# matheusfalcaopinto/triple-hybrid-rag

Measured on AMD Instinct MI355X. Metric: queries/sec (fused top-10), higher is better.
Workload: dtype f16 MFMA shortlist scan (f32 accumulate) + f64 rescoring of the f32 rows; 1 GPU; 1000000-doc / 768-d dense-only brute-force cosine top-10 (BASELINE.json configs[1]); pipeline=dense, docs=1000000, dim=768, semantic_top_k=100, fused_top_k=10, shortlist=f16, parallelism=single GPU, world_size_seen=1, rescued_queries=0

## Files before the change

### triple-hybrid-rag_amd/csrc/dense_scan_f16q.hpp

```cpp
#pragma once
#include "dense_common.hpp"

namespace thr {

constexpr int Q_RING = 4;
constexpr int Q_NW = 4;

template <int DIM>
struct QScan {
    static constexpr int KS = DIM / 16;
    static constexpr int HS = KS / 2;
    static constexpr int HALF_BYTES = HS * 1024;
    static constexpr int PER_CU = DIM <= 768 ? 2 : 1;
    static constexpr int NB = (160 * 1024 / PER_CU) / HALF_BYTES > 4 ? 4 : (160 * 1024 / PER_CU) / HALF_BYTES;
    static constexpr int PER = HS / Q_NW;
#ifndef THR_Q_RING_1024
#define THR_Q_RING_1024 8
#endif
    static constexpr int RING = PER_CU == 1 ? THR_Q_RING_1024 : Q_RING;
#ifdef Q_PROBE_EXTRA
    static constexpr int VM_PER_PIECE = 2, LDS_BYTES = NB * HALF_BYTES + 32 * 1024;
#else
    static constexpr int VM_PER_PIECE = 1, LDS_BYTES = NB * HALF_BYTES;
#endif
    static_assert(HS % Q_NW == 0 && NB >= 3, "half tile must split evenly over the waves; >= 3 buffers");
};

template <int DIM, int SHAPE>
__global__ __launch_bounds__(256) void pack_queries_f16(const float* __restrict__ queries,
                                                        int n_queries, f32x4* __restrict__ qfrag,
                                                        float* __restrict__ qerr) {
    constexpr int KS = DIM / 16;
    const int lane = threadIdx.x & 63, wave = threadIdx.x >> 6;
    __shared__ double red[4][4][32];
    double e = 0.0, nn = 0.0, e_hi = 0.0, n_hi = 0.0;
#pragma unroll 4
    for (int s = wave; s < KS; s += 4) {
        int q, d0;
        if constexpr (SHAPE == 32) {
            q = blockIdx.x * 32 + (lane & 31);
            d0 = 16 * s + 8 * (lane >> 5);
        } else {
            q = blockIdx.x * 32 + 16 * (s / (KS / 2)) + (lane & 15);
            d0 = 32 * (s % (KS / 2)) + 8 * (lane >> 4);
        }
        f32x4 lo = {0.f, 0.f, 0.f, 0.f}, hi = lo;
        if (q < n_queries) {
            const f32x4* src = reinterpret_cast<const f32x4*>(queries + (int64_t)q * DIM + d0);
            lo = src[0];
            hi = src[1];
        }
        const f32x4 packed = pack_f16x8(lo, hi);
        qfrag[((int64_t)blockIdx.x * KS + s) * 64 + lane] = packed;
        const half8 hv = __builtin_bit_cast(half8, packed);
        double e1 = 0.0, n1 = 0.0;
#pragma unroll
        for (int j = 0; j < 8; ++j) {
            const float v = j < 4 ? lo[j] : hi[j - 4];
            const double d = (double)v - (double)(float)hv[j];
            e1 += d * d;
            n1 += (double)v * (double)v;
        }
        if (SHAPE == 32 || s < KS / 2) {
            e += e1;
            nn += n1;
        } else {
            e_hi += e1;
            n_hi += n1;
        }
    }
    if constexpr (SHAPE == 32) {
        e += __shfl_xor(e, 32, WAVE);
        nn += __shfl_xor(nn, 32, WAVE);
        if (lane < 32) {
            red[wave][0][lane] = e;
            red[wave][1][lane] = nn;
        }
    } else {
#pragma unroll
        for (int m = 16; m <= 32; m <<= 1) {
            e += __shfl_xor(e, m, WAVE);
            nn += __shfl_xor(nn, m, WAVE);
            e_hi += __shfl_xor(e_hi, m, WAVE);
            n_hi += __shfl_xor(n_hi, m, WAVE);
        }
        if (lane < 16) {
            red[wave][0][lane] = e;
            red[wave][1][lane] = nn;
            red[wave][0][16 + lane] = e_hi;
            red[wave][1][16 + lane] = n_hi;
        }
    }
    __syncthreads();
    if (threadIdx.x < 32) {
        double es = 0.0, ns = 0.0;
#pragma unroll
        for (int w = 0; w < 4; ++w) {
            es += red[w][0][threadIdx.x];
            ns += red[w][1][threadIdx.x];
        }
        const float rel = ns > 0.0 ? (float)sqrt(es / ns) : 0.f;
        qerr[blockIdx.x * 32 + threadIdx.x] = __uint_as_float(__float_as_uint(rel) + 1u);
    }
}

#define QS_RD(dst, ks) \
    asm volatile("ds_read_b128 %0, %1 offset:%2" : "=v"(dst) : "v"(abase), "n"((ks) * 1024) : "memory")
template <int S, int HS, int RING>
__device__ __forceinline__ void qs_fill(f32x4 (&a)[RING], uint32_t abase) {
    if constexpr (S < RING && S < HS) {
        QS_RD(a[S], S);
        qs_fill<S + 1, HS>(a, abase);
    }
}
template <int SHAPE>
struct QAcc;
template <>
struct QAcc<32> {
    static constexpr int NQL = 1, SEGS = 2;
    static constexpr int QW = 32, NQB = 2, NREG = 16;
    f32x16 v;
    __device__ __forceinline__ void zero() {
#pragma unroll
        for (int x = 0; x < 16; ++x) v[x] = 0.f;
    }
    template <int X> __device__ __forceinline__ float get() const { return v[X]; }
    template <int X> static __device__ __forceinline__ int row(int lane) { return (X & 3) + 8 * (X >> 2) + 4 * (lane >> 5); }
    template <int X> static constexpr int qsel() { return 0; }
    static __device__ __forceinline__ int query(int lane, int) { return lane & 31; }
    static __device__ __forceinline__ int seg(int lane) { return lane >> 5; }
};
template <>
struct QAcc<48> {
    static constexpr int NQL = 3, SEGS = 4;
    static constexpr int QW = 48, NQB = 3, NREG = 24;
    f32x4 t[6];
    __device__ __forceinline__ void zero() {
#pragma unroll
        for (int x = 0; x < 6; ++x) t[x] = f32x4{0.f, 0.f, 0.f, 0.f};
    }
    template <int X> __device__ __forceinline__ float get() const { return t[X >> 2][X & 3]; }
    template <int X> static __device__ __forceinline__ int row(int lane) { return 16 * ((X >> 2) / 3) + 4 * (lane >> 4) + (X & 3); }
    template <int X> static constexpr int qsel() { return (X >> 2) % 3; }
    static __device__ __forceinline__ int query(int lane, int qb) { return 16 * qb + (lane & 15); }
    static __device__ __forceinline__ int seg(int lane) { return lane >> 4; }
};
template <>
struct QAcc<16> {
    static constexpr int NQL = 2, SEGS = 4;
    static constexpr int QW = 32, NQB = 2, NREG = 16;
    f32x4 t[4];
    __device__ __forceinline__ void zero() {
#pragma unroll
        for (int x = 0; x < 4; ++x) t[x] = f32x4{0.f, 0.f, 0.f, 0.f};
    }
    template <int X> __device__ __forceinline__ float get() const { return t[X >> 2][X & 3]; }
    template <int X> static __device__ __forceinline__ int row(int lane) { return 16 * (X >> 3) + 4 * (lane >> 4) + (X & 3); }
    template <int X> static constexpr int qsel() { return (X >> 2) & 1; }
    static __device__ __forceinline__ int query(int lane, int qb) { return 16 * qb + (lane & 15); }
    static __device__ __forceinline__ int seg(int lane) { return lane >> 4; }
};

template <int S, int K0, int KS, int SHAPE, int NBQ>
__device__ __forceinline__ void qsx_mfma(const f32x4& a, const f32x4 (&bq)[NBQ], QAcc<SHAPE>& acc) {
    if constexpr (SHAPE == 32) {
        acc.v = __builtin_amdgcn_mfma_f32_32x32x16_f16(__builtin_bit_cast(half8, a),
                                                       __builtin_bit_cast(half8, bq[K0 + S]), acc.v, 0, 0, 0);
    } else {
        constexpr int k32 = (K0 + S) / 2, ra = S & 1, NQB = QAcc<SHAPE>::NQB;
        static_assert(NBQ == NQB * KS / 2, "one B fragment per 16-query block and 32-dim step");
        static_for<0, NQB>([&](auto qb) {
            acc.t[NQB * ra + qb] = __builtin_amdgcn_mfma_f32_16x16x32_f16(
                __builtin_bit_cast(half8, a), __builtin_bit_cast(half8, bq[qb * (KS / 2) + k32]),
                acc.t[NQB * ra + qb], 0, 0, 0);
        });
    }
}
template <int S, int HS, int K0, int KS, int PER, int SHAPE, int RING, int NBQ, typename Issue>
__device__ __forceinline__ void qsx_steps(f32x4 (&a)[RING], const f32x4 (&bq)[NBQ], QAcc<SHAPE>& acc,
                                          uint32_t abase, Issue& issue_piece) {
    if constexpr (S < HS) {
        constexpr int left = HS - S - 1 < RING - 1 ? HS - S - 1 : RING - 1;
        asm volatile("s_waitcnt lgkmcnt(%1)" : "+v"(a[S % RING]) : "n"(left) : "memory");
        qsx_mfma<S, K0, KS, SHAPE>(a[S % RING], bq, acc);
        if constexpr (S + RING < HS) QS_RD(a[S % RING], S + RING);
        constexpr int every = HS / PER;
        if constexpr (S % every == 1 && S / every < PER) issue_piece(std::integral_constant<int, S / every>{});
        qsx_steps<S + 1, HS, K0, KS, PER, SHAPE, RING, NBQ>(a, bq, acc, abase, issue_piece);
    }
}

template <int NQL, bool COLL>
struct QColl {
    const int32_t* doc_coll;
    int qc[NQL];
};
template <int NQL>
struct QColl<NQL, false> {};

template <int SHAPE, bool COLL>
struct QEmit : QColl<QAcc<SHAPE>::NQL, COLL> {
    static constexpr int NQL = QAcc<SHAPE>::NQL;
    const Cand* cand;
    float tau[NQL];
    uint32_t slot[NQL], end[NQL];
    template <int X>
    __device__ __forceinline__ void one(const QAcc<SHAPE>& acc, uint32_t row0, int lane) {
        constexpr int qs = QAcc<SHAPE>::template qsel<X>();
        const float v = acc.template get<X>();
        if (v >= tau[qs]) {
            const uint32_t row = row0 + (uint32_t)QAcc<SHAPE>::template row<X>(lane);
            if constexpr (COLL) {
                if (this->qc[qs] != -1 && this->doc_coll[row] != this->qc[qs]) return;
            }
            if (slot[qs] < end[qs]) {
                const uint64_t word = (uint64_t)__float_as_uint(v) | ((uint64_t)row << 32);
                asm volatile("global_store_dwordx2 %0, %1, %2" ::"v"(slot[qs]), "v"(word), "s"(cand) : "memory");
            }
            slot[qs] += 8;
        }
    }
    template <int X>
    __device__ __forceinline__ void all(const QAcc<SHAPE>& acc, uint32_t row0, int lane) {
        if constexpr (X < QAcc<SHAPE>::NREG) {
            one<X>(acc, row0, lane);
            all<X + 1>(acc, row0, lane);
        }
    }
};

template <int SHAPE, bool COLL>
struct QTop : QColl<QAcc<SHAPE>::NQL, COLL> {
    static constexpr int NQL = QAcc<SHAPE>::NQL;
    float t[NQL][SAMPLE_TOP];
    __device__ __forceinline__ void init() {
#pragma unroll
        for (int u = 0; u < NQL; ++u)
#pragma unroll
            for (int j = 0; j < SAMPLE_TOP; ++j) t[u][j] = -INFINITY;
    }
    template <int X>
    __device__ __forceinline__ void one(const QAcc<SHAPE>& acc, uint32_t row0, int lane) {
        constexpr int qs = QAcc<SHAPE>::template qsel<X>();
        float x = acc.template get<X>();
        x = x == x ? x : -INFINITY;
        if constexpr (COLL) {
            if (this->doc_coll && this->qc[qs] != -1 && x > -INFINITY) {
                const uint32_t row = row0 + (uint32_t)QAcc<SHAPE>::template row<X>(lane);
                if (this->doc_coll[row] != this->qc[qs]) x = -INFINITY;
            }
        }
#pragma unroll
        for (int j = 0; j < SAMPLE_TOP; ++j) {
            const float hi = fmaxf(t[qs][j], x);
            x = fminf(t[qs][j], x);
            t[qs][j] = hi;
        }
    }
    template <int X>
    __device__ __forceinline__ void all(const QAcc<SHAPE>& acc, uint32_t row0, int lane) {
        if constexpr (X < QAcc<SHAPE>::NREG) {
            one<X>(acc, row0, lane);
            all<X + 1>(acc, row0, lane);
        }
    }
    __device__ __forceinline__ void store(float* __restrict__ sample, int u, int64_t q, int nseg, int seg) const {
        float* dst = sample + (q * nseg + seg) * SAMPLE_TOP;
#pragma unroll
        for (int j = 0; j < SAMPLE_TOP; ++j) dst[j] = t[u][j];
    }
};

template <int S, int HS, int K0, int KS, int PER, int SHAPE, int HF, int RING, int NBQ, bool COLL, typename Issue>
__device__ __forceinline__ void qsx_steps_pe(f32x4 (&a)[RING], const f32x4 (&bq)[NBQ], QAcc<SHAPE>& acc,
                                             uint32_t abase, Issue& issue_piece, QEmit<SHAPE, COLL>& em,
                                             const QAcc<SHAPE>& prv, uint32_t row_prv, int lane) {
    if constexpr (S < HS) {
        constexpr int left = HS - S - 1 < RING - 1 ? HS - S - 1 : RING - 1;
        asm volatile("s_waitcnt lgkmcnt(%1)" : "+v"(a[S % RING]) : "n"(left) : "memory");
        qsx_mfma<S, K0, KS, SHAPE>(a[S % RING], bq, acc);
        if constexpr (S + RING < HS) QS_RD(a[S % RING], S + RING);
        constexpr int every = HS / PER;
        if constexpr (S % every == 1 && S / every < PER) issue_piece(std::integral_constant<int, S / every>{});
        constexpr int NRH = QAcc<SHAPE>::NREG / 2, j = S * NRH / HS;
        if constexpr ((S + 1) * NRH / HS > j) em.template one<NRH * HF + j>(prv, row_prv, lane);
        qsx_steps_pe<S + 1, HS, K0, KS, PER, SHAPE, HF, RING, NBQ, COLL>(a, bq, acc, abase, issue_piece, em, prv, row_prv, lane);
    }
}
#undef QS_RD

template <int DIM, int MODE, bool PROF = false, int SHAPE = 32, bool COLL = true>
__global__ __launch_bounds__(Q_NW * 64, QScan<DIM>::PER_CU) void dense_scan_f16q(
    const f32x4* __restrict__ packed, const f32x4* __restrict__ qfrag, int n_qtiles,
    int64_t n_tiles, int64_t tile_stride, const float* __restrict__ tau,
    int* __restrict__ seg_cnt, Cand* __restrict__ cand, int seg_cap,
    float* __restrict__ sample,
    const int32_t* __restrict__ doc_coll, const int32_t* __restrict__ query_coll, int n_queries,
    unsigned long long* __restrict__ stamps = nullptr) {
    using C = QScan<DIM>;
    using A = QAcc<SHAPE>;
    constexpr int KS = C::KS, HS = C::HS, NB = C::NB, PER = C::PER, NQL = A::NQL, QW = A::QW;
    constexpr int NBQ = SHAPE == 32 ? KS : A::NQB * KS / 2;
    extern __shared__ f32x4 lds_rows[];

    const ScanSlot slot = scan_slot(n_qtiles);
    const int lane = threadIdx.x & 63;
    const int wave = __builtin_amdgcn_readfirstlane(threadIdx.x >> 6);
    const int q32 = slot.qtile * Q_NW + wave;
    const bool idle = (int64_t)q32 * QW >= n_queries;

    f32x4 bq[NBQ];
    if (!idle)
        static_for<0, NBQ>([&](auto s) {
            bq[s] = qfrag[((int64_t)q32 * NBQ + s) * 64 + lane];
        });
    const int nseg = A::SEGS * slot.nslices;
    const int my_seg = A::SEGS * slot.slice + A::seg(lane);
    QEmit<SHAPE, COLL> em;
    em.cand = cand;
    QTop<SHAPE, COLL> top;
    if constexpr (COLL) em.doc_coll = top.doc_coll = doc_coll;
    top.init();
    uint32_t start[NQL];
#pragma unroll
    for (int u = 0; u < NQL; ++u) {
        const int q = q32 * QW + A::query(lane, u);
        em.tau[u] = MODE == MODE_FILTER ? tau[q] : 0.f;
        if constexpr (COLL) em.qc[u] = top.qc[u] = (query_coll && q < n_queries) ? query_coll[q] : -1;
        start[u] = (uint32_t)(((int64_t)q * CAND_CAP + (int64_t)my_seg * seg_cap) * sizeof(Cand));
        em.slot[u] = start[u];
        em.end[u] = start[u] + (uint32_t)(seg_cap * sizeof(Cand));
    }
    __builtin_amdgcn_s_waitcnt(0x0F70);

    const int64_t first = slot.slice, step = slot.nslices;
    const int64_t n_mine = first < n_tiles ? (n_tiles - first + step - 1) / step : 0;
    const int64_t n_half = 2 * n_mine;
    const uint32_t lds_base = (uint32_t)(size_t)(__attribute__((address_space(3))) void*)lds_rows;
    auto piece_src = [&](int64_t j) -> const f32x4* {
        const int64_t jc = j < n_half ? j : n_half - 1;
        const int64_t t = first + (jc >> 1) * step;
        return packed + ((t * tile_stride * KS + (jc & 1) * HS + wave) * 64 + lane);
    };
#ifdef Q_PROBE_EXTRA
    f32x4 probe_reg = {0.f, 0.f, 0.f, 0.f};
#endif
    auto dma = [&](const f32x4* src, int buf, int p) {
        __builtin_amdgcn_global_load_lds(
            (const __attribute__((address_space(1))) void*)(src + p * Q_NW * 64),
            (__attribute__((address_space(3))) void*)(size_t)(lds_base + buf * C::HALF_BYTES +
                                                              (wave + p * Q_NW) * 1024),
            16, 0, 0);
#ifdef Q_PROBE_EXTRA
        const uint32_t scratch = lds_base + NB * C::HALF_BYTES + (wave + (p & 7) * Q_NW) * 1024;
        if constexpr (Q_PROBE_EXTRA == 1) {
            __builtin_amdgcn_global_load_lds(
                (const __attribute__((address_space(1))) void*)(src + p * Q_NW * 64),
                (__attribute__((address_space(3))) void*)(size_t)scratch, 16, 0, 0);
        } else {
            asm volatile("ds_write_b128 %0, %1" ::"v"(scratch + lane * 16), "v"(probe_reg) : "memory");
            asm volatile("global_load_dwordx4 %0, %1, off" : "=v"(probe_reg) : "v"(src + p * Q_NW * 64) : "memory");
        }
#endif
    };
    if (n_half > 0) {
#pragma unroll
        for (int b = 0; b < NB - 1; ++b) {
            const f32x4* src = piece_src(b);
#pragma unroll
            for (int p = 0; p < PER; ++p) dma(src, b, p);
        }
    }

    unsigned long long ph[5] = {0, 0, 0, 0, 0}, t_loop = 0, t_prev = 0;
    auto stamp = [&](int j) {
        if constexpr (PROF) {
            const unsigned long long t = __builtin_amdgcn_s_memtime();
            if (j >= 0) ph[j] += t - t_prev;
            t_prev = t;
        }
    };
    if constexpr (PROF) t_loop = __builtin_amdgcn_s_memtime();

    A acc;
    int buf = 0;
    if (idle) {
#pragma unroll 1
        for (int64_t j = 0; j < n_half; ++j) {
            asm volatile("s_waitcnt vmcnt(%0)" ::"n"((NB - 2) * PER * C::VM_PER_PIECE) : "memory");
            __builtin_amdgcn_s_barrier();
            const int nbuf = buf == 0 ? NB - 1 : buf - 1;
            const f32x4* src = piece_src(j + NB - 1);
#pragma unroll
            for (int p = 0; p < PER; ++p) dma(src, nbuf, p);
            buf = buf + 1 == NB ? 0 : buf + 1;
        }
    }
#ifdef Q_NO_PIPE_EMIT
    constexpr bool PIPE_EMIT = false;
#else
    constexpr bool PIPE_EMIT = true;
#endif
    if constexpr (PIPE_EMIT && MODE == MODE_FILTER && !PROF && C::PER_CU == 1 && SHAPE != 48) {
        A acc2[2];
#pragma unroll
        for (int x = 0; x < A::NREG; ++x) {
            if constexpr (SHAPE == 32) acc2[1].v[x] = -INFINITY;
            else acc2[1].t[x >> 2][x & 3] = -INFINITY;
        }
        uint32_t row_of[2] = {0u, 0u};
#define QS_HALF_PE(hf, CUR, PRV)                                                                   \
    {                                                                                              \
        asm volatile("s_waitcnt vmcnt(%0)" ::"n"((NB - 2) * PER * C::VM_PER_PIECE) : "memory");                      \
        __builtin_amdgcn_s_barrier();                                                              \
        const int nbuf = buf == 0 ? NB - 1 : buf - 1;                  \
        const f32x4* src = piece_src(2 * i + (hf) + NB - 1);                                       \
        auto issue_piece = [&](auto P) { dma(src, nbuf, decltype(P)::value); };                    \
        const uint32_t abase = lds_base + buf * C::HALF_BYTES + lane * 16;                         \
        f32x4 a[C::RING];                                                                           \
        qs_fill<0, HS>(a, abase);                                                                  \
        qsx_steps_pe<0, HS, (hf) * HS, KS, PER, SHAPE, (hf)>(a, bq, acc2[CUR], abase, issue_piece, \
                                                            em, acc2[PRV], row_of[PRV], lane);     \
        buf = buf + 1 == NB ? 0 : buf + 1;                                                         \
    }
        const int64_t n_it = idle ? 0 : n_mine;
        int64_t i = 0;
#pragma unroll 1
        for (; i + 1 < n_it; i += 2) {
            acc2[0].zero();
            QS_HALF_PE(0, 0, 1)
            QS_HALF_PE(1, 0, 1)
            row_of[0] = (uint32_t)((first + i * step) * tile_stride * 32);
            ++i;
            acc2[1].zero();
            QS_HALF_PE(0, 1, 0)
            QS_HALF_PE(1, 1, 0)
            row_of[1] = (uint32_t)((first + i * step) * tile_stride * 32);
            --i;
        }
        if (i < n_it) {
            acc2[0].zero();
            QS_HALF_PE(0, 0, 1)
            QS_HALF_PE(1, 0, 1)
            em.template all<0>(acc2[0], (uint32_t)((first + i * step) * tile_stride * 32), lane);
        } else if (n_it > 0) {
            em.template all<0>(acc2[1], row_of[1], lane);
        }
#undef QS_HALF_PE
    } else {
#pragma unroll 1
    for (int64_t i = 0; i < (idle ? 0 : n_mine); ++i) {
#define QS_HALF(hf)                                                                                \
    {                                                                                              \
        stamp(-1);                                                                                 \
               \
        asm volatile("s_waitcnt vmcnt(%0)" ::"n"((NB - 2) * PER * C::VM_PER_PIECE) : "memory");                      \
        stamp(0);                                                                                  \
        __builtin_amdgcn_s_barrier();                                                              \
        stamp(1);                                                                                  \
        const int nbuf = buf == 0 ? NB - 1 : buf - 1;                  \
        const f32x4* src = piece_src(2 * i + (hf) + NB - 1);                                       \
        auto issue_piece = [&](auto P) { dma(src, nbuf, decltype(P)::value); };                    \
        const uint32_t abase = lds_base + buf * C::HALF_BYTES + lane * 16;                         \
        f32x4 a[C::RING];                                                                           \
        qs_fill<0, HS>(a, abase);                                                                  \
        stamp(2);                                                                                  \
        qsx_steps<0, HS, (hf) * HS, KS, PER, SHAPE>(a, bq, acc, abase, issue_piece);                \
        if constexpr (PROF) {                                                                      \
            if constexpr (SHAPE == 32) asm volatile("" : "+v"(acc.v));                               \
            else {                                                                                 \
                asm volatile("" : "+v"(acc.t[0]), "+v"(acc.t[1]), "+v"(acc.t[2]), "+v"(acc.t[3]));   \
                if constexpr (A::NQB == 3) asm volatile("" : "+v"(acc.t[4]), "+v"(acc.t[5]));       \
            }                                                                                      \
        }                                                                                          \
        stamp(3);                                                                                  \
        buf = buf + 1 == NB ? 0 : buf + 1;                                                         \
    }
        acc.zero();
        QS_HALF(0)
        QS_HALF(1)
#undef QS_HALF

        const int64_t t = first + i * step;
        if constexpr (MODE == MODE_ALL) {
            top.template all<0>(acc, (uint32_t)(t * tile_stride * 32), lane);
        } else {
            em.template all<0>(acc, (uint32_t)(t * tile_stride * 32), lane);
        }
        stamp(4);
    }
    }
    asm volatile("s_waitcnt vmcnt(0)" ::: "memory");
    if constexpr (MODE == MODE_FILTER) {
#pragma unroll
        for (int u = 0; u < NQL; ++u)
            seg_cnt[(int64_t)(q32 * QW + A::query(lane, u)) * nseg + my_seg] = (int)((em.slot[u] - start[u]) / sizeof(Cand));
    } else {
#pragma unroll
        for (int u = 0; u < NQL; ++u) top.store(sample, u, (int64_t)q32 * QW + A::query(lane, u), nseg, my_seg);
    }
    if constexpr (PROF) {
        if (lane == 0) {
            unsigned long long* o = stamps + ((int64_t)blockIdx.x * Q_NW + wave) * 8;
            for (int j = 0; j < 5; ++j) o[j] = ph[j];
            o[5] = (unsigned long long)n_half;
            o[6] = __builtin_amdgcn_s_memtime() - t_loop;
            o[7] = (unsigned long long)__builtin_amdgcn_s_getreg((4 << 0) | (0 << 6) | (31 << 11));
        }
    }
}

constexpr int QS_NW = 8;
constexpr int QS_NBUF = 6;

template <int DIM>
struct QStag {
    static constexpr int KS = DIM / 16, HS = KS / 2, HALF_BYTES = HS * 1024;
    static constexpr int PER = HS / QS_NW;
    static constexpr int LDS_BYTES = QS_NBUF * HALF_BYTES;
    static_assert(HS % QS_NW == 0 && LDS_BYTES <= 160 * 1024, "dim 512 / 768 only");
};

template <int DIM, int MODE, int SHAPE = 32, bool COLL = true>
__global__ __launch_bounds__(QS_NW * 64) void dense_scan_f16qs(
    const f32x4* __restrict__ packed, const f32x4* __restrict__ qfrag, int n_qtiles,
    int64_t n_tiles, int64_t tile_stride, const float* __restrict__ tau,
    int* __restrict__ seg_cnt, Cand* __restrict__ cand, int seg_cap,
    float* __restrict__ sample,
    const int32_t* __restrict__ doc_coll, const int32_t* __restrict__ query_coll, int n_queries) {
    using C = QStag<DIM>;
    using A = QAcc<SHAPE>;
    constexpr int KS = C::KS, HS = C::HS, PER = C::PER, NBUF = QS_NBUF, NQL = A::NQL;
    extern __shared__ f32x4 lds_rows[];

    const ScanSlot slot = scan_slot(n_qtiles);
    const int lane = threadIdx.x & 63;
    const int wave = __builtin_amdgcn_readfirstlane(threadIdx.x >> 6);
    const int q32 = slot.qtile * QS_NW + wave;

    f32x4 bq[KS];
    if ((int64_t)q32 * 32 < n_queries)
        static_for<0, KS>([&](auto s) {
            bq[s] = qfrag[((int64_t)q32 * KS + s) * 64 + lane];
        });
    const int nseg = A::SEGS * slot.nslices;
    const int my_seg = A::SEGS * slot.slice + A::seg(lane);
    QEmit<SHAPE, COLL> em;
    em.cand = cand;
    QTop<SHAPE, COLL> top;
    if constexpr (COLL) em.doc_coll = top.doc_coll = doc_coll;
    top.init();
    uint32_t start[NQL];
#pragma unroll
    for (int u = 0; u < NQL; ++u) {
        const int q = q32 * 32 + A::query(lane, u);
        em.tau[u] = MODE == MODE_FILTER ? tau[q] : 0.f;
        if constexpr (COLL) em.qc[u] = top.qc[u] = (query_coll && q < n_queries) ? query_coll[q] : -1;
        start[u] = (uint32_t)(((int64_t)q * CAND_CAP + (int64_t)my_seg * seg_cap) * sizeof(Cand));
        em.slot[u] = start[u];
        em.end[u] = start[u] + (uint32_t)(seg_cap * sizeof(Cand));
    }
    __builtin_amdgcn_s_waitcnt(0x0F70);

    const int64_t first = slot.slice, step = slot.nslices;
    const int64_t n_mine = first < n_tiles ? (n_tiles - first + step - 1) / step : 0;
    const int64_t n_half = 2 * n_mine;
    const uint32_t lds_base = (uint32_t)(size_t)(__attribute__((address_space(3))) void*)lds_rows;
    auto piece_src = [&](int64_t j) -> const f32x4* {
        const int64_t jc = j < n_half ? j : n_half - 1;
        const int64_t t = first + (jc >> 1) * step;
        return packed + ((t * tile_stride * KS + (jc & 1) * HS + wave) * 64 + lane);
    };
    auto dma = [&](const f32x4* src, int buf, int p) {
        __builtin_amdgcn_global_load_lds(
            (const __attribute__((address_space(1))) void*)(src + p * QS_NW * 64),
            (__attribute__((address_space(3))) void*)(size_t)(lds_base + buf * C::HALF_BYTES +
                                                              (wave + p * QS_NW) * 1024),
            16, 0, 0);
    };
#define QS_EMIT(i_)                                                                                \
    if constexpr (MODE == MODE_ALL) {                                                              \
        top.template all<0>(acc, (uint32_t)((first + (i_) * step) * tile_stride * 32), lane);      \
    } else {                                                                                       \
        em.template all<0>(acc, (uint32_t)((first + (i_) * step) * tile_stride * 32), lane);       \
    }
#define QS_SYNC()                                                      \
    asm volatile("s_waitcnt vmcnt(%0)" ::"n"(3 * PER) : "memory");     \
    __builtin_amdgcn_s_barrier();

    if (n_half > 0) {
#pragma unroll
        for (int b = 0; b < 4; ++b) {
            const f32x4* src = piece_src(b);
#pragma unroll
            for (int p = 0; p < PER; ++p) dma(src, b, p);
        }
    }
    A acc;
    f32x4 a[Q_RING];
    if ((int64_t)q32 * 32 >= n_queries) {
        int buf = wave < 4 ? 4 : 5;
        int64_t j = wave < 4 ? 4 : 5;
        if (wave >= 4) {
            QS_SYNC()
            if (n_half > 0) {
                const f32x4* src = piece_src(4);
#pragma unroll
                for (int p = 0; p < PER; ++p) dma(src, 4, p);
            }
        }
#pragma unroll 1
        for (int64_t k = 0; k < n_half; ++k, ++j) {
            QS_SYNC()
            const f32x4* src = piece_src(j);
#pragma unroll
            for (int p = 0; p < PER; ++p) dma(src, buf, p);
            buf = buf + 1 == NBUF ? 0 : buf + 1;
        }
        if (wave < 4) {
            QS_SYNC()
        }
    } else if (wave < 4) {
        int buf = 0;
#pragma unroll 1
        for (int64_t i = 0; i < n_mine; ++i) {
            {
                QS_SYNC()
                const int nbuf = buf + 4 >= NBUF ? buf + 4 - NBUF : buf + 4;
                const f32x4* src = piece_src(2 * i + 4);
                auto issue_piece = [&](auto P) { dma(src, nbuf, decltype(P)::value); };
                const uint32_t abase = lds_base + buf * C::HALF_BYTES + lane * 16;
                qs_fill<0, HS>(a, abase);
                acc.zero();
                qsx_steps<0, HS, 0, KS, PER, SHAPE>(a, bq, acc, abase, issue_piece);
                buf = buf + 1 == NBUF ? 0 : buf + 1;
            }
            {
                QS_SYNC()
                const int nbuf = buf + 4 >= NBUF ? buf + 4 - NBUF : buf + 4;
                const f32x4* src = piece_src(2 * i + 5);
                auto issue_piece = [&](auto P) { dma(src, nbuf, decltype(P)::value); };
                const uint32_t abase = lds_base + buf * C::HALF_BYTES + lane * 16;
                qs_fill<0, HS>(a, abase);
                qsx_steps<0, HS, HS, KS, PER, SHAPE>(a, bq, acc, abase, issue_piece);
                buf = buf + 1 == NBUF ? 0 : buf + 1;
            }
            QS_EMIT(i)
        }
        QS_SYNC()
    } else {
        QS_SYNC()
        if (n_half > 0) {
            const f32x4* src = piece_src(4);
#pragma unroll
            for (int p = 0; p < PER; ++p) dma(src, 4, p);
        }
        int buf = 0;
#pragma unroll 1
        for (int64_t i = 0; i < n_mine; ++i) {
            const int buf1 = buf + 1 == NBUF ? 0 : buf + 1;
            const int buf2 = buf1 + 1 == NBUF ? 0 : buf1 + 1;
            {
                QS_SYNC()
                if (i > 0) {
                    QS_EMIT(i - 1)
                }
                const int nbuf = buf + 5 >= NBUF ? buf + 5 - NBUF : buf + 5;
                const f32x4* src = piece_src(2 * i + 5);
                auto issue_piece = [&](auto P) { dma(src, nbuf, decltype(P)::value); };
                const uint32_t abase = lds_base + buf * C::HALF_BYTES + lane * 16;
                if (i == 0) qs_fill<0, HS>(a, abase);
                acc.zero();
                qsx_steps<0, HS, 0, KS, PER, SHAPE>(a, bq, acc, abase, issue_piece);
                qs_fill<0, HS>(a, lds_base + buf1 * C::HALF_BYTES + lane * 16);
            }
            {
                QS_SYNC()
                const f32x4* src = piece_src(2 * i + 6);
                auto issue_piece = [&](auto P) { dma(src, buf, decltype(P)::value); };
                const uint32_t abase = lds_base + buf1 * C::HALF_BYTES + lane * 16;
                qsx_steps<0, HS, HS, KS, PER, SHAPE>(a, bq, acc, abase, issue_piece);
                if (i + 1 < n_mine)
                    qs_fill<0, HS>(a, lds_base + buf2 * C::HALF_BYTES + lane * 16);
            }
            buf = buf2;
        }
        if (n_mine > 0) {
            QS_EMIT(n_mine - 1)
        }
    }
#undef QS_SYNC
#undef QS_EMIT
    asm volatile("s_waitcnt vmcnt(0)" ::: "memory");
    if constexpr (MODE == MODE_FILTER) {
#pragma unroll
        for (int u = 0; u < NQL; ++u)
            seg_cnt[(int64_t)(q32 * 32 + A::query(lane, u)) * nseg + my_seg] = (int)((em.slot[u] - start[u]) / sizeof(Cand));
    } else {
#pragma unroll
        for (int u = 0; u < NQL; ++u) top.store(sample, u, (int64_t)q32 * 32 + A::query(lane, u), nseg, my_seg);
    }
}

__global__ __launch_bounds__(256) void quantize_f16_norm(const float* __restrict__ docs,
                                                         int64_t n_docs, int dim, int shape,
                                                         _Float16* __restrict__ packed,
                                                         unsigned int* __restrict__ max_err_bits) {
    const int lane = threadIdx.x & 63;
    const int64_t row = (int64_t)blockIdx.x * (blockDim.x / WAVE) + (threadIdx.x >> 6);
    const int64_t n_pad = (n_docs + 31) / 32 * 32;
    if (row >= n_pad) return;
    const int64_t tile = row >> 5;
    const int r = (int)(row & 31), ks = dim / 16;
    const float* x = docs + row * dim;
    double nn = 0.0;
    if (row < n_docs)
        for (int i = lane; i < dim; i += WAVE) nn += (double)x[i] * (double)x[i];
    for (int m = 32; m >= 1; m >>= 1) nn += __shfl_xor(nn, m, WAVE);
    const double dn = sqrt(nn);
    const bool live = dn > 0.0;
    double err = 0.0;
    for (int i = lane; i < dim; i += WAVE) {
        const float v = live ? x[i] : 0.f;
        const _Float16 hv = live ? (_Float16)(float)((double)v / dn) : (_Float16)__builtin_nanf("");
        if (packed) {
            if (shape == 32) {
                const int s = i >> 4, hh = (i >> 3) & 1, e = i & 7;
                packed[(((tile * ks + s) * 64) + r + 32 * hh) * 8 + e] = hv;
            } else {
                const int k32 = i >> 5, g = (i >> 3) & 3, e = i & 7, ra = r >> 4;
                packed[(((tile * ks + 2 * k32 + ra) * 64) + (r & 15) + 16 * g) * 8 + e] = hv;
            }
        }
        if (live) {
            const double d = (double)v / dn - (double)(float)hv;
            err += d * d;
        }
    }
    for (int m = 32; m >= 1; m >>= 1) err += __shfl_xor(err, m, WAVE);
    if (lane == 0 && live) {
        float rel = (float)sqrt(err);
        rel = __uint_as_float(__float_as_uint(rel) + 1u);
        atomicMax(max_err_bits, __float_as_uint(rel));
    }
}

__global__ __launch_bounds__(256) void measure_f16_error(const float* __restrict__ docs, int64_t n_docs,
                                                         int dim, unsigned int* __restrict__ max_rel_bits) {
    const int lane = threadIdx.x & 63;
    const int64_t row = (int64_t)blockIdx.x * (blockDim.x / WAVE) + (threadIdx.x >> 6);
    if (row >= n_docs) return;
    const float* x = docs + row * dim;
    double err = 0.0, nrm = 0.0;
    for (int i = lane; i < dim; i += WAVE) {
        const float v = x[i];
        const double d = (double)v - (double)(float)(_Float16)v;
        err += d * d;
        nrm += (double)v * (double)v;
    }
    for (int m = 32; m >= 1; m >>= 1) {
        err += __shfl_xor(err, m, WAVE);
        nrm += __shfl_xor(nrm, m, WAVE);
    }
    if (lane == 0 && nrm > 0.0) {
        float rel = (float)sqrt(err / nrm);
        rel = __uint_as_float(__float_as_uint(rel) + 1u);
        atomicMax(max_rel_bits, __float_as_uint(rel));
    }
}

}
```

Before: 790,900 queries/s.

## Restructure staggered f16 scan around whole-tile buffers with dedicated issuer waves

Reworks the 8-wave staggered scan kernel so each LDS buffer holds a whole tile instead of a half, with one barrier per tile instead of two. Only waves 4-7 issue global-to-LDS DMA, spreading the pieces across their MFMA steps, while waves 0-3 only multiply. The schedule (buffer count, prologue depth, vmcnt wait depth) moves into a new constexpr helper header. This halves barrier count and simplifies buffer rotation, at the cost of fewer LDS buffers (4 full tiles vs 6 halves) and an uneven DMA load between wave groups.

```diff
diff --git a/triple-hybrid-rag_amd/csrc/dense_scan_f16q.hpp b/triple-hybrid-rag_amd/csrc/dense_scan_f16q.hpp
--- a/triple-hybrid-rag_amd/csrc/dense_scan_f16q.hpp
+++ b/triple-hybrid-rag_amd/csrc/dense_scan_f16q.hpp
@@ -1,5 +1,6 @@
 #pragma once
 #include "dense_common.hpp"
+#include "dense_tile_schedule.hpp"
 
 namespace thr {
 
@@ -285,6 +286,19 @@
         constexpr int NRH = QAcc<SHAPE>::NREG / 2, j = S * NRH / HS;
         if constexpr ((S + 1) * NRH / HS > j) em.template one<NRH * HF + j>(prv, row_prv, lane);
         qsx_steps_pe<S + 1, HS, K0, KS, PER, SHAPE, HF, RING, NBQ, COLL>(a, bq, acc, abase, issue_piece, em, prv, row_prv, lane);
+    }
+}
+template <int S, int KS, int PB, int SHAPE, int RING, int NBQ, typename Issue>
+__device__ __forceinline__ void qst_steps(f32x4 (&a)[RING], const f32x4 (&bq)[NBQ], QAcc<SHAPE>& acc,
+                                          uint32_t abase, Issue& issue_piece) {
+    if constexpr (S < KS) {
+        constexpr int left = KS - S - 1 < RING - 1 ? KS - S - 1 : RING - 1;
+        asm volatile("s_waitcnt lgkmcnt(%1)" : "+v"(a[S % RING]) : "n"(left) : "memory");
+        qsx_mfma<S, 0, KS, SHAPE>(a[S % RING], bq, acc);
+        if constexpr (S + RING < KS) QS_RD(a[S % RING], S + RING);
+        constexpr int p = (S - 1) / 2;
+        if constexpr (S >= 1 && p < PB && tsched::issue_step(p) == S) issue_piece(std::integral_constant<int, p>{});
+        qst_steps<S + 1, KS, PB, SHAPE, RING, NBQ>(a, bq, acc, abase, issue_piece);
     }
 }
 #undef QS_RD
@@ -510,15 +524,16 @@
     }
 }
 
-constexpr int QS_NW = 8;
-constexpr int QS_NBUF = 6;
+constexpr int QS_NW = tsched::N_WAVES;
 
 template <int DIM>
 struct QStag {
-    static constexpr int KS = DIM / 16, HS = KS / 2, HALF_BYTES = HS * 1024;
-    static constexpr int PER = HS / QS_NW;
-    static constexpr int LDS_BYTES = QS_NBUF * HALF_BYTES;
-    static_assert(HS % QS_NW == 0 && LDS_BYTES <= 160 * 1024, "dim 512 / 768 only");
+    static constexpr int KS = tsched::pieces_per_tile(DIM), TILE_BYTES = tsched::tile_bytes(DIM);
+    static constexpr int NBUF = tsched::nbuf(DIM);
+    static constexpr int PB = tsched::pieces_issued(tsched::ROLE_B, DIM);
+    static constexpr int LDS_BYTES = NBUF * TILE_BYTES;
+    static_assert(KS % tsched::N_ISSUERS == 0 && NBUF >= 3 && LDS_BYTES <= tsched::LDS_BUDGET, "dim 512 / 768 only");
+    static_assert(tsched::wait_leaves(tsched::ROLE_B, DIM) < 64 && tsched::issue_step(PB - 1) < KS, "vmcnt is 6 bits");
 };
 
 template <int DIM, int MODE, int SHAPE = 32, bool COLL = true>
@@ -530,7 +545,7 @@
     const int32_t* __restrict__ doc_coll, const int32_t* __restrict__ query_coll, int n_queries) {
     using C = QStag<DIM>;
     using A = QAcc<SHAPE>;
-    constexpr int KS = C::KS, HS = C::HS, PER = C::PER, NBUF = QS_NBUF, NQL = A::NQL;
+    constexpr int KS = C::KS, PB = C::PB, NQL = A::NQL;
     extern __shared__ f32x4 lds_rows[];
 
     const ScanSlot slot = scan_slot(n_qtiles);
@@ -562,20 +577,21 @@
     }
     __builtin_amdgcn_s_waitcnt(0x0F70);
 
+    namespace ts = tsched;
     const int64_t first = slot.slice, step = slot.nslices;
     const int64_t n_mine = first < n_tiles ? (n_tiles - first + step - 1) / step : 0;
-    const int64_t n_half = 2 * n_mine;
     const uint32_t lds_base = (uint32_t)(size_t)(__attribute__((address_space(3))) void*)lds_rows;
+    const ts::Role role = ts::role_of(wave, (int64_t)q32 * 32 >= n_queries);
+    const int iw = wave & (ts::N_ISSUERS - 1);
     auto piece_src = [&](int64_t j) -> const f32x4* {
-        const int64_t jc = j < n_half ? j : n_half - 1;
-        const int64_t t = first + (jc >> 1) * step;
-        return packed + ((t * tile_stride * KS + (jc & 1) * HS + wave) * 64 + lane);
+        const int64_t t = first + ts::source_tile(j, n_mine) * step;
+        return packed + ((t * tile_stride * KS + iw) * 64 + lane);
     };
     auto dma = [&](const f32x4* src, int buf, int p) {
         __builtin_amdgcn_global_load_lds(
-            (const __attribute__((address_space(1))) void*)(src + p * QS_NW * 64),
-            (__attribute__((address_space(3))) void*)(size_t)(lds_base + buf * C::HALF_BYTES +
-                                                              (wave + p * QS_NW) * 1024),
+            (const __attribute__((address_space(1))) void*)(src + (ts::piece_index(iw, p) - iw) * 64),
+            (__attribute__((address_space(3))) void*)(size_t)(lds_base + buf * C::TILE_BYTES +
+                                                              ts::piece_index(iw, p) * 1024),
             16, 0, 0);
     };
 #define QS_EMIT(i_)                                                                                \
@@ -584,112 +600,74 @@
     } else {                                                                                       \
         em.template all<0>(acc, (uint32_t)((first + (i_) * step) * tile_stride * 32), lane);       \
     }
-#define QS_SYNC()                                                      \
-    asm volatile("s_waitcnt vmcnt(%0)" ::"n"(3 * PER) : "memory");     \
+    constexpr int WAIT_B = ts::wait_leaves(ts::ROLE_B, DIM);
+    static_assert(WAIT_B == ts::wait_leaves(ts::ROLE_PAD_B, DIM) && ts::pieces_issued(ts::ROLE_PAD_B, DIM) == PB &&
+                  ts::pieces_issued(ts::ROLE_A, DIM) == 0 && ts::pieces_issued(ts::ROLE_PAD_A, DIM) == 0,
+                  "a padding wave moves what a working wave of its group moves");
+#define QS_SYNC_B()                                                    \
+    asm volatile("s_waitcnt vmcnt(%0)" ::"n"(WAIT_B) : "memory");      \
     __builtin_amdgcn_s_barrier();
 
-    if (n_half > 0) {
-#pragma unroll
-        for (int b = 0; b < 4; ++b) {
+    if (ts::issues(role) && n_mine > 0) {
+#pragma unroll
+        for (int b = 0; b < ts::prologue_tiles(DIM); ++b) {
             const f32x4* src = piece_src(b);
 #pragma unroll
-            for (int p = 0; p < PER; ++p) dma(src, b, p);
+            for (int p = 0; p < PB; ++p) dma(src, ts::buffer_of(b, DIM), p);
         }
     }
     A acc;
     f32x4 a[Q_RING];
-    if ((int64_t)q32 * 32 >= n_queries) {
-        int buf = wave < 4 ? 4 : 5;
-        int64_t j = wave < 4 ? 4 : 5;
-        if (wave >= 4) {
-            QS_SYNC()
-            if (n_half > 0) {
-                const f32x4* src = piece_src(4);
-#pragma unroll
-                for (int p = 0; p < PER; ++p) dma(src, 4, p);
+    auto no_piece = [](auto) {};
+    if (!ts::multiplies(role)) {
+        if (ts::issues(role)) {
+            int ibuf = ts::buffer_of(ts::issue_tile(0, DIM), DIM);
+#pragma unroll 1
+            for (int64_t t = 0; t < ts::barriers(ts::ROLE_PAD_B, n_mine); ++t) {
+                QS_SYNC_B()
+                const f32x4* src = piece_src(ts::issue_tile(t, DIM));
+#pragma unroll
+                for (int p = 0; p < PB; ++p) dma(src, ibuf, p);
+                ibuf = ts::next_buffer(ibuf, DIM);
             }
-        }
+        } else {
 #pragma unroll 1
-        for (int64_t k = 0; k < n_half; ++k, ++j) {
-            QS_SYNC()
-            const f32x4* src = piece_src(j);
-#pragma unroll
-            for (int p = 0; p < PER; ++p) dma(src, buf, p);
-            buf = buf + 1 == NBUF ? 0 : buf + 1;
-        }
-        if (wave < 4) {
-            QS_SYNC()
-        }
-    } else if (wave < 4) {
+            for (int64_t t = 0; t < ts::barriers(ts::ROLE_PAD_A, n_mine); ++t) __builtin_amdgcn_s_barrier();
+        }
+    } else if (role == ts::ROLE_A) {
         int buf = 0;
 #pragma unroll 1
-        for (int64_t i = 0; i < n_mine; ++i) {
-            {
-                QS_SYNC()
-                const int nbuf = buf + 4 >= NBUF ? buf + 4 - NBUF : buf + 4;
-                const f32x4* src = piece_src(2 * i + 4);
-                auto issue_piece = [&](auto P) { dma(src, nbuf, decltype(P)::value); };
-                const uint32_t abase = lds_base + buf * C::HALF_BYTES + lane * 16;
-                qs_fill<0, HS>(a, abase);
-                acc.zero();
-                qsx_steps<0, HS, 0, KS, PER, SHAPE>(a, bq, acc, abase, issue_piece);
-                buf = buf + 1 == NBUF ? 0 : buf + 1;
-            }
-            {
-                QS_SYNC()
-                const int nbuf = buf + 4 >= NBUF ? buf + 4 - NBUF : buf + 4;
-                const f32x4* src = piece_src(2 * i + 5);
-                auto issue_piece = [&](auto P) { dma(src, nbuf, decltype(P)::value); };
-                const uint32_t abase = lds_base + buf * C::HALF_BYTES + lane * 16;
-                qs_fill<0, HS>(a, abase);
-                qsx_steps<0, HS, HS, KS, PER, SHAPE>(a, bq, acc, abase, issue_piece);
-                buf = buf + 1 == NBUF ? 0 : buf + 1;
-            }
+        for (int64_t i = 0; i < ts::barriers(ts::ROLE_A, n_mine); ++i) {
+            __builtin_amdgcn_s_barrier();
+            const uint32_t abase = lds_base + buf * C::TILE_BYTES + lane * 16;
+            qs_fill<0, KS>(a, abase);
+            acc.zero();
+            qst_steps<0, KS, 0, SHAPE>(a, bq, acc, abase, no_piece);
+            buf = ts::next_buffer(buf, DIM);
             QS_EMIT(i)
         }
-        QS_SYNC()
     } else {
-        QS_SYNC()
-        if (n_half > 0) {
-            const f32x4* src = piece_src(4);
-#pragma unroll
-            for (int p = 0; p < PER; ++p) dma(src, 4, p);
-        }
         int buf = 0;
 #pragma unroll 1
-        for (int64_t i = 0; i < n_mine; ++i) {
-            const int buf1 = buf + 1 == NBUF ? 0 : buf + 1;
-            const int buf2 = buf1 + 1 == NBUF ? 0 : buf1 + 1;
-            {
-                QS_SYNC()
-                if (i > 0) {
-                    QS_EMIT(i - 1)
-                }
-                const int nbuf = buf + 5 >= NBUF ? buf + 5 - NBUF : buf + 5;
-                const f32x4* src = piece_src(2 * i + 5);
-                auto issue_piece = [&](auto P) { dma(src, nbuf, decltype(P)::value); };
-                const uint32_t abase = lds_base + buf * C::HALF_BYTES + lane * 16;
-                if (i == 0) qs_fill<0, HS>(a, abase);
-                acc.zero();
-                qsx_steps<0, HS, 0, KS, PER, SHAPE>(a, bq, acc, abase, issue_piece);
-                qs_fill<0, HS>(a, lds_base + buf1 * C::HALF_BYTES + lane * 16);
+        for (int64_t i = 0; i < ts::barriers(ts::ROLE_B, n_mine); ++i) {
+            QS_SYNC_B()
+            if (i > 0) {
+                QS_EMIT(i - 1)
             }
-            {
-                QS_SYNC()
-                const f32x4* src = piece_src(2 * i + 6);
-                auto issue_piece = [&](auto P) { dma(src, buf, decltype(P)::value); };
-                const uint32_t abase = lds_base + buf1 * C::HALF_BYTES + lane * 16;
-                qsx_steps<0, HS, HS, KS, PER, SHAPE>(a, bq, acc, abase, issue_piece);
-                if (i + 1 < n_mine)
-                    qs_fill<0, HS>(a, lds_base + buf2 * C::HALF_BYTES + lane * 16);
-            }
-            buf = buf2;
+            const int ibuf = ts::prev_buffer(buf, DIM);
+            const f32x4* src = piece_src(ts::issue_tile(i, DIM));
+            auto issue_piece = [&](auto P) { dma(src, ibuf, decltype(P)::value); };
+            const uint32_t abase = lds_base + buf * C::TILE_BYTES + lane * 16;
+            qs_fill<0, KS>(a, abase);
+            acc.zero();
+            qst_steps<0, KS, PB, SHAPE>(a, bq, acc, abase, issue_piece);
+            buf = ts::next_buffer(buf, DIM);
         }
         if (n_mine > 0) {
             QS_EMIT(n_mine - 1)
         }
     }
-#undef QS_SYNC
+#undef QS_SYNC_B
 #undef QS_EMIT
     asm volatile("s_waitcnt vmcnt(0)" ::: "memory");
     if constexpr (MODE == MODE_FILTER) {
diff --git a/triple-hybrid-rag_amd/csrc/dense_tile_schedule.hpp b/triple-hybrid-rag_amd/csrc/dense_tile_schedule.hpp
--- /dev/null
+++ b/triple-hybrid-rag_amd/csrc/dense_tile_schedule.hpp
@@ -0,0 +1,45 @@
+#pragma once
+#include <cstdint>
+
+#if defined(__HIPCC__) || defined(__CUDACC__)
+#define THR_TS_FN constexpr __host__ __device__ inline
+#else
+#define THR_TS_FN constexpr inline
+#endif
+
+namespace thr {
+namespace tsched {
+
+enum Role { ROLE_A = 0, ROLE_B = 1, ROLE_PAD_A = 2, ROLE_PAD_B = 3 };
+constexpr int N_ROLES = 4;
+constexpr int N_WAVES = 8, N_ISSUERS = 4;
+constexpr int LDS_BUDGET = 160 * 1024, MAX_BUF = 4;
+
+THR_TS_FN Role role_of(int wave, bool padding) {
+    return wave < N_WAVES - N_ISSUERS ? (padding ? ROLE_PAD_A : ROLE_A) : (padding ? ROLE_PAD_B : ROLE_B);
+}
+THR_TS_FN int pieces_per_tile(int dim) { return dim / 16; }
+THR_TS_FN int tile_bytes(int dim) { return pieces_per_tile(dim) * 1024; }
+THR_TS_FN int nbuf(int dim) {
+    return LDS_BUDGET / tile_bytes(dim) > MAX_BUF ? MAX_BUF : LDS_BUDGET / tile_bytes(dim);
+}
+THR_TS_FN bool issues(Role r) { return r == ROLE_B || r == ROLE_PAD_B; }
+THR_TS_FN bool multiplies(Role r) { return r == ROLE_A || r == ROLE_B; }
+THR_TS_FN bool emits_first(Role r) { return r == ROLE_B; }
+THR_TS_FN int pieces_issued(Role r, int dim) { return issues(r) ? pieces_per_tile(dim) / N_ISSUERS : 0; }
+THR_TS_FN int piece_index(int iw, int p) { return iw + N_ISSUERS * p; }
+THR_TS_FN int issue_step(int p) { return 1 + 2 * p; }
+
+THR_TS_FN int buffer_of(int64_t tile, int dim) { return (int)(tile % nbuf(dim)); }
+THR_TS_FN int next_buffer(int buf, int dim) { return buf + 1 == nbuf(dim) ? 0 : buf + 1; }
+THR_TS_FN int prev_buffer(int buf, int dim) { return buf == 0 ? nbuf(dim) - 1 : buf - 1; }
+THR_TS_FN int prologue_tiles(int dim) { return nbuf(dim) - 1; }
+THR_TS_FN int64_t issue_tile(int64_t t, int dim) { return t + nbuf(dim) - 1; }
+THR_TS_FN int64_t source_tile(int64_t j, int64_t n_mine) { return j < n_mine ? j : n_mine - 1; }
+THR_TS_FN int64_t read_tile(Role, int64_t t) { return t; }
+THR_TS_FN int wait_leaves(Role r, int dim) { return (nbuf(dim) - 2) * pieces_issued(r, dim); }
+THR_TS_FN bool waits(Role r) { return issues(r); }
+THR_TS_FN int64_t barriers(Role, int64_t n_mine) { return n_mine; }
+
+}
+}
```

Result: faster. 829,100 queries/s, median of 6 (+4.8%).
